# jkk-research/urban_road_filter

Hardware: NVIDIA H100
Metric: scans_per_sec (higher is better)
Workload: dtype f32/f64

## Files before the change

urban_road_filter_b200/csrc/urf_api.cu:

```cuda
#include <algorithm>
#include <cmath>
#include <cstdio>
#include <cstdlib>
#include <cstring>
#include <string>
#include <vector>

#include "urf_kernels.cuh"
#include "urf_host.hpp"
#include "urf_queue_internal.hpp"

using namespace urf;

constexpr int kMaxBatch = 65535;

struct urf_ctx {
  int device = 0;
  int max_points = 0;
  int max_batch = 0;
  size_t P = 0;
  int Tmax = 0;
  cudaStream_t stream = nullptr;
  cudaStream_t s_in = nullptr, s_out = nullptr;
  static constexpr int kGroups = 16;
  cudaStream_t s_grp[kGroups] = {};
  cudaEvent_t ev_fork = nullptr, ev_join[kGroups] = {};
  cudaStream_t s_side[kGroups + 1] = {};
  cudaEvent_t ev_sfork[kGroups + 1] = {}, ev_sjoin[kGroups + 1] = {};
  int sort_ctas = 0;
  int groups = 2;
  bool use_graph = true;
  cudaGraphExec_t gexec = nullptr;
  int g_B = -1, g_S = -1, g_order = -1, g_launches = 0;
  unsigned long long g_version = 0, version = 1;
  std::vector<cudaEvent_t> ev_in, ev_comp;
  cudaEvent_t ev0 = nullptr, ev1 = nullptr;
  DevBuffers buf{};
  struct HostSlot {
    float4* in = nullptr;
    unsigned char* rawb = nullptr;
    size_t rawb_bytes = 0;
    int* n = nullptr;
    int* label = nullptr;
    signed char* label8 = nullptr;
    int* order = nullptr;
    int* ring = nullptr;
    ScanOut* out = nullptr;
    int* h_n = nullptr;
    ScanOut* h_out = nullptr;
    cudaEvent_t ev0 = nullptr, ev1 = nullptr;
    cudaEvent_t ev_done = nullptr;
    int batch = 0, S = 0, launches = 0;
    urf_result* outs = nullptr;
    urf_clouds* clouds = nullptr;
  };
  HostSlot hs[2];
  int hs_head = 0, hs_count = 0;
  float4* pack = nullptr;
  int* packcnt = nullptr;
  int* packtot = nullptr;
  int tie_order = URF_TIES_INPUT_ORDER;
  int* h_packtot = nullptr;
  urf_params params{};
  DevParams dp{};
  static constexpr int kNRing = 8;
  int* h_nring = nullptr;
  cudaEvent_t ev_nring[kNRing] = {};
  int nring_pos = 0;
  int last_B = 0, last_S = 0;
  int launches = 0;
  float last_ms = 0.f;
  bool timing_valid = false, timing_host = false;
  std::string err;
  std::vector<void*> allocs;
  bool profile = false;
  int kslots = 1, kslot = 0;
  std::vector<cudaEvent_t> kev;
  std::vector<const char*> knames;
  std::vector<int> kcounts;
  int kcount = 0;
};

namespace {

int cuda_rc(urf_ctx* ctx, cudaError_t e, const char* call) {
  if (e == cudaSuccess) return URF_OK;
  ctx->err = std::string(call) + ": " + cudaGetErrorString(e);
  return e == cudaErrorMemoryAllocation ? URF_ERR_NOMEM : URF_ERR_CUDA;
}

#define CK(call)                                                                                   \
  do {                                                                                             \
    const int rc_ = cuda_rc(ctx, (call), #call);                                                   \
    if (rc_ != URF_OK) return rc_;                                                                 \
  } while (0)

template <class T> int dalloc(urf_ctx* ctx, T** p, size_t count) {
  void* q = nullptr;
  CK(cudaMalloc(&q, count * sizeof(T) + 256));
  ctx->allocs.push_back(q);
  CK(cudaMemsetAsync(q, 0, count * sizeof(T) + 256, ctx->stream));
  CK(cudaStreamSynchronize(ctx->stream));
  *p = static_cast<T*>(q);
  return URF_OK;
}

__global__ void k_ring32(DevBuffers buf, int* dst, int S) {
  const int b = blockIdx.y, i = blockIdx.x * blockDim.x + threadIdx.x;
  if (i < buf.n[b]) dst[(size_t)b * S + i] = max((int)buf.ringid[(size_t)b * S + i], -1);
}

DevBuffers offset_view(const DevBuffers& a, int b0, int S, int T, int channels) {
  DevBuffers v = a;
  const size_t o = (size_t)b0 * S;
  v.in += o; v.label += o; v.order += o; v.n += b0; v.out += b0;
  if (v.epos) { v.epos += o; v.lomuto += (size_t)b0 * (kRingKeys + 1); }
  if (v.label8) v.label8 += o;
  v.alpha_v += o; v.mark += o; v.ringid += o; v.sect += o; v.bpt += o;
  v.sr += o; v.sz += o; v.sidx += o; v.ssrz += o; v.ssl += o;
  v.az += o; v.d2 += o; v.baz += o; v.roadlist += o; v.roadcnt += (size_t)b0 * ((S + 31) >> 5); v.sortbuf += 2 * o;
  v.Tf += (size_t)b0 * channels * kTStride; v.Tb += (size_t)b0 * channels * kTStride;
  v.lut += (size_t)b0 * (kElevBins + 1); v.firstidx += (size_t)b0 * (kElevBins + 1);
  v.hist += (size_t)b0 * T * channels;
  v.cmin += (size_t)b0 * channels * kDegBins; v.cmax += (size_t)b0 * channels * kDegBins;
  v.ne += (size_t)b0 * channels * (kDegBins + 1);
  v.tab += b0;
  return v;
}

constexpr int kMaxKernels = 32;
constexpr int kMarkSingleMax = 300000;
thread_local std::string g_create_err;

int launch_pipeline(urf_ctx* ctx, const DevBuffers& buf, int B, int S, bool want_order, int group, int* launched) {
  DevParams dp = ctx->dp;
  const bool ref = ctx->tie_order == URF_TIES_REFERENCE;
  dp.want_order = want_order || ref ? 1 : 0;
  cudaStream_t st = group < urf_ctx::kGroups ? ctx->s_grp[group] : ctx->stream;
  const int T = (S + kChunk - 1) / kChunk;
  if (T > ctx->Tmax) return URF_ERR_CAPACITY;
  int L = 0;
  ctx->kcount = 0;
  const dim3 gpts((S + 255) / 256, B), gchunk((T + kWarpsPerBlock - 1) / kWarpsPerBlock, B);
#define K(name, ...)                                                                         \
  do {                                                                                       \
    if (ctx->profile && ctx->kcount < kMaxKernels) {                                         \
      ctx->knames[ctx->kcount] = name;                                                       \
      CK(cudaEventRecord(ctx->kev[(size_t)ctx->kslot * (kMaxKernels + 1) + ctx->kcount], st)); \
      ctx->kcount++;                                                                         \
    }                                                                                        \
    __VA_ARGS__;                                                                             \
    L++;                                                                                     \
  } while (0)
  K("k_reset", k_reset<<<dim3(8, B), 256, 0, st>>>(buf, dp));
  K("k_points", k_points<<<gpts, 256, 0, st>>>(buf, dp, S));
  K("k_register", k_register<<<B, 256, 0, st>>>(buf, dp, S));
  K("k_assign", k_assign<<<gchunk, kWarpsPerBlock * 32, 0, st>>>(buf, dp, S, T));
  K("k_scan_offsets", k_scan_offsets<<<B, kScanOffThreads, 0, st>>>(buf, dp, S, T));
  K("k_scatter", k_scatter<<<dim3((T + kScatterWarps - 1) / kScatterWarps, B), kScatterWarps * 32, kScatterSmem, st>>>(buf, dp, S, T));
  const bool fork = dp.star && !ctx->profile;
  cudaStream_t st_ring = fork ? ctx->s_side[group] : st;
  if (fork) {
    CK(cudaEventRecord(ctx->ev_sfork[group], st));
    CK(cudaStreamWaitEvent(st_ring, ctx->ev_sfork[group], 0));
  }
  if (dp.curbPoints == 5)
    K("k_ring_detect4", k_ring_detect4<<<dim3((S + kTile4 - 1) / kTile4, B), 256, 0, st_ring>>>(buf, dp, S));
  else K("k_ring_detect", k_ring_detect<<<gpts, 256, 0, st_ring>>>(buf, dp, S));
  if (fork) CK(cudaEventRecord(ctx->ev_sjoin[group], st_ring));
  if (dp.star) {
    const int gbig = std::max(4, std::min(kSectKeys, 2048 / B));
    const dim3 gscan((kSectKeys + kScanWarps * 32 - 1) / (kScanWarps * 32), B);
    const int gsort = std::min(ctx->sort_ctas, (B * kSectKeys + kSortWarps - 1) / kSortWarps);
    K("k_star_sort", k_star_sort<<<gsort, kSortWarps * 32, kStarSortSmem, st>>>(buf, dp, S, B));
    K("k_star_sort_big", k_star_sort_big<<<dim3(gbig, B), 256, kStarCtaSmem, st>>>(buf, dp, S));
    K("k_star_scan", k_star_scan<<<gscan, kScanWarps * 32, 0, st>>>(buf, dp, S));
    if (dp.star_prefix)
      K("k_star_refine", k_star_refine<<<dim3(std::max(8, std::min(kSectKeys / 8, 8192 / B)), B), 256, kStarCtaSmem, st>>>(buf, dp, S));
  }
  if (fork) CK(cudaStreamWaitEvent(st, ctx->ev_sjoin[group], 0));
  K("k_tab1", k_tab1<<<dim3((dp.channels + 7) / 8, B), 256, 0, st>>>(buf, dp));
  K("k_reach", k_reach<<<dim3((2 * kDegBins + 7) / 8, B), 256, 0, st>>>(buf, dp));
  K("k_tab2", k_tab2<<<dim3((dp.channels + kTab2Rings - 1) / kTab2Rings, B), kTab2Rings * 64, 0, st>>>(buf, dp));
  const dim3 glabel((S + kLabelThreads * kLabelGroups - 1) / (kLabelThreads * kLabelGroups), B), gsort(dp.channels, B);
  if (ref) {
    K("k_sort_rings", k_sort_rings<true><<<gsort, kSortThreads, kRingSmemKeys * sizeof(unsigned long long), st>>>(buf, S));
    K("k_lomuto_rings", k_lomuto_rings<<<gsort, kLomutoThreads, kLomutoSmem, st>>>(buf, S));
    K("k_label", k_label<true><<<glabel, kLabelThreads, 0, st>>>(buf, dp, S));
  } else K("k_label", k_label<false><<<glabel, kLabelThreads, 0, st>>>(buf, dp, S));
  if (S > kMarkSingleMax) {
    const dim3 gm(std::max(1, std::min(64, S / 16384)), B);
    K("k_markers_grid1", k_markers_grid<1><<<gm, kMarkGridThreads, 0, st>>>(buf, S));
    K("k_markers_grid2", k_markers_grid<2><<<gm, kMarkGridThreads, 0, st>>>(buf, S));
    if (ref) K("k_verts", k_verts<true><<<B, 384, 0, st>>>(buf, S));
    else K("k_verts", k_verts<false><<<B, 384, 0, st>>>(buf, S));
  } else if (ref) K("k_markers1", k_markers1<true><<<dim3(1, B), kMark1Threads, 0, st>>>(buf, S));
  else K("k_markers1", k_markers1<false><<<dim3(1, B), kMark1Threads, 0, st>>>(buf, S));
  if (want_order && !ref) K("k_sort_rings", k_sort_rings<false><<<gsort, kSortThreads, kRingSmemKeys * sizeof(unsigned long long), st>>>(buf, S));
#undef K
  if (ctx->profile) {
    CK(cudaEventRecord(ctx->kev[(size_t)ctx->kslot * (kMaxKernels + 1) + kMaxKernels], st));
    ctx->kcounts[ctx->kslot] = ctx->kcount;
    ctx->kslot = (ctx->kslot + 1) % ctx->kslots;
  }
  CK(cudaGetLastError());
  *launched = L;
  return URF_OK;
}

int update_graph(urf_ctx* ctx, int B, int S, bool want_order) {
  if (ctx->gexec && ctx->g_B == B && ctx->g_S == S && ctx->g_order == (int)want_order && ctx->g_version == ctx->version) return URF_OK;
  if (ctx->gexec) { cudaGraphExecDestroy(ctx->gexec); ctx->gexec = nullptr; }
  cudaGraph_t graph = nullptr;
  CK(cudaStreamBeginCapture(ctx->stream, cudaStreamCaptureModeThreadLocal));
  int L = 0;
  const int rc = launch_pipeline(ctx, ctx->buf, B, S, want_order, urf_ctx::kGroups, &L);
  const cudaError_t e = cudaStreamEndCapture(ctx->stream, &graph);
  if (rc != URF_OK || e != cudaSuccess || !graph) { if (graph) cudaGraphDestroy(graph); ctx->err = "graph capture failed"; return rc != URF_OK ? rc : URF_ERR_CUDA; }
  const cudaError_t ei = cudaGraphInstantiate(&ctx->gexec, graph, 0);
  cudaGraphDestroy(graph);
  if (ei != cudaSuccess) { ctx->gexec = nullptr; ctx->err = cudaGetErrorString(ei); return URF_ERR_CUDA; }
  ctx->g_B = B; ctx->g_S = S; ctx->g_order = (int)want_order; ctx->g_version = ctx->version; ctx->g_launches = L;
  return URF_OK;
}

void fill_result(const ScanOut& o, urf_result* r, bool with_ring_start) {
  r->n_in = o.n_in; r->n_roi = o.n_roi;
  r->flags = o.flags & F_PUBLIC_MASK; r->reserved = 0;
  if (o.n_roi < 30) {
    r->status = URF_TOO_FEW_POINTS;
    r->n_rings = 0; r->n_order = 0; r->n_road = 0; r->n_curb = 0; r->n_vert = 0;
    if (with_ring_start && r->ring_start) for (int k = 0; k <= URF_MAX_CHANNELS; k++) r->ring_start[k] = 0;
    return;
  }
  r->status = URF_OK;
  r->n_rings = o.n_rings; r->n_order = o.n_order; r->n_road = o.n_road; r->n_curb = o.n_curb; r->n_vert = o.n_vert;
  std::memcpy(r->vert, o.vert, sizeof(float) * 4 * (size_t)o.n_vert);
  if (with_ring_start && r->ring_start) std::memcpy(r->ring_start, o.ring_start, sizeof(int) * (URF_MAX_CHANNELS + 1));
}

}

extern "C" {

int urf_version(void) { return URF_VERSION; }

const char* urf_strerror(int code) {
  switch (code) {
    case URF_OK: return "ok";
    case URF_TOO_FEW_POINTS: return "fewer than 30 points in the ROI: nothing published";
    case URF_ERR_INVALID: return "invalid argument";
    case URF_ERR_NO_DEVICE: return "no CUDA device (this library has no CPU fallback)";
    case URF_ERR_CUDA: return "CUDA error";
    case URF_ERR_NOMEM: return "out of device or pinned memory";
    case URF_ERR_CAPACITY: return "scan or batch larger than the context was created for";
    case URF_ERR_TIMEOUT: return "timed out";
    case URF_ERR_CLOSED: return "queue closed";
    default: return "unknown error";
  }
}

const char* urf_last_cuda_error(const urf_ctx* ctx) {
  if (ctx) return ctx->err.c_str();
  return g_create_err.empty() ? "null context" : g_create_err.c_str();
}

void urf_default_params(urf_params* p) {
  if (!p) return;
  std::memset(p, 0, sizeof(*p));
  std::snprintf(p->fixed_frame, sizeof(p->fixed_frame), "left_os1/os1_lidar");
  std::snprintf(p->topic_name, sizeof(p->topic_name), "/left_os1/os1_cloud_node/points");
  p->x_zero_method = 1; p->z_zero_method = 1; p->star_shaped_method = 1; p->blind_spots = 1; p->xDirection = 0;
  p->interval = 0.18; p->curb_height = 0.05; p->curb_points = 5; p->beamZone = 30;
  p->min_x = 0; p->max_x = 30; p->min_y = -10; p->max_y = 10; p->min_z = -3; p->max_z = -1;
  p->cylinder_deg_x = 150; p->cylinder_deg_z = 140; p->curb_slope_deg = 50;
  p->kdev_param = 1.225; p->kdist_param = 2; p->starbeam_filter = 0; p->dmin_param = 10;
  p->simple_poly_allow = 1; p->poly_s_param = 0.7; p->poly_z_manual = -1.5; p->poly_z_avg_allow = 1;
  p->channels = 64;
}

int urf_create(urf_ctx** out, int device, int max_points, int max_batch) {
  if (!out || max_points < 1 || max_batch < 1 || max_points > (1 << 24)) return URF_ERR_INVALID;
  if ((long long)(max_points + kChunk) * max_batch >= (1ll << 31)) return URF_ERR_CAPACITY;
  if (max_batch > kMaxBatch) return URF_ERR_CAPACITY;
  *out = nullptr;
  int ndev = 0;
  if (cudaGetDeviceCount(&ndev) != cudaSuccess || ndev <= 0 || device < 0 || device >= ndev) return URF_ERR_NO_DEVICE;
  urf_ctx* ctx = new urf_ctx();
  auto fail = [&](int rc) { g_create_err = ctx->err.empty() ? std::string(urf_strerror(rc)) : ctx->err; urf_destroy(ctx); return rc; };
  ctx->device = device;
  if (cudaSetDevice(device) != cudaSuccess) return fail(URF_ERR_NO_DEVICE);
  ctx->max_points = ((max_points + kChunk - 1) / kChunk) * kChunk;
  ctx->max_batch = max_batch;
  ctx->P = (size_t)ctx->max_points * max_batch;
  ctx->Tmax = ctx->max_points / kChunk;
  int rc;
#define TRY(x) do { rc = (x); if (rc != URF_OK) return fail(rc); } while (0)
#define CKF(call) do { cudaError_t e_ = (call); if (e_ != cudaSuccess) { ctx->err = cudaGetErrorString(e_); return fail(URF_ERR_CUDA); } } while (0)
  CKF(cudaStreamCreateWithFlags(&ctx->stream, cudaStreamNonBlocking));
  CKF(cudaStreamCreateWithFlags(&ctx->s_in, cudaStreamNonBlocking));
  CKF(cudaStreamCreateWithFlags(&ctx->s_out, cudaStreamNonBlocking));
  for (int g = 0; g < urf_ctx::kGroups; g++) {
    CKF(cudaStreamCreateWithFlags(&ctx->s_grp[g], cudaStreamNonBlocking));
    CKF(cudaEventCreateWithFlags(&ctx->ev_join[g], cudaEventDisableTiming));
  }
  CKF(cudaEventCreateWithFlags(&ctx->ev_fork, cudaEventDisableTiming));
  for (int g = 0; g <= urf_ctx::kGroups; g++) {
    CKF(cudaStreamCreateWithFlags(&ctx->s_side[g], cudaStreamNonBlocking));
    CKF(cudaEventCreateWithFlags(&ctx->ev_sfork[g], cudaEventDisableTiming));
    CKF(cudaEventCreateWithFlags(&ctx->ev_sjoin[g], cudaEventDisableTiming));
  }
  CKF(cudaEventCreate(&ctx->ev0));
  CKF(cudaEventCreate(&ctx->ev1));
  const size_t P = ctx->P;
  DevBuffers& b = ctx->buf;
  urf_ctx::HostSlot& h0 = ctx->hs[0];
  TRY(dalloc(ctx, &h0.in, P));
  h0.rawb_bytes = (size_t)ctx->max_points * URF_MAX_POINT_STEP;
  TRY(dalloc(ctx, &h0.rawb, h0.rawb_bytes));
  TRY(dalloc(ctx, &b.alpha_v, P));
  TRY(dalloc(ctx, &b.mark, P));
  TRY(dalloc(ctx, &b.ringid, P));
  TRY(dalloc(ctx, &b.sect, P));
  TRY(dalloc(ctx, &h0.label, P));
  TRY(dalloc(ctx, &b.bpt, P));
  TRY(dalloc(ctx, &b.sr, P));
  TRY(dalloc(ctx, &b.sz, P));
  TRY(dalloc(ctx, &b.sidx, P));
  TRY(dalloc(ctx, &b.ssrz, P));
  TRY(dalloc(ctx, &b.ssl, P));
  TRY(dalloc(ctx, &b.az, P));
  TRY(dalloc(ctx, &b.d2, P));
  TRY(dalloc(ctx, &b.baz, P));
  TRY(dalloc(ctx, &b.roadlist, P));
  TRY(dalloc(ctx, &b.roadcnt, P / 32 + (size_t)max_batch + 1));
  TRY(dalloc(ctx, &b.Tf, (size_t)max_batch * kTStride * URF_MAX_CHANNELS));
  TRY(dalloc(ctx, &b.Tb, (size_t)max_batch * kTStride * URF_MAX_CHANNELS));
  TRY(dalloc(ctx, &b.lut, (size_t)max_batch * (kElevBins + 1)));
  TRY(dalloc(ctx, &b.order, P));
  TRY(dalloc(ctx, &b.sortbuf, 2 * P));
  TRY(dalloc(ctx, &b.hist, (size_t)max_batch * ctx->Tmax * kRingKeys));
  TRY(dalloc(ctx, &b.firstidx, (size_t)max_batch * (kElevBins + 1)));
  TRY(dalloc(ctx, &b.cmin, (size_t)max_batch * URF_MAX_CHANNELS * kDegBins));
  TRY(dalloc(ctx, &b.cmax, (size_t)max_batch * URF_MAX_CHANNELS * kDegBins));
  TRY(dalloc(ctx, &b.ne, (size_t)max_batch * URF_MAX_CHANNELS * (kDegBins + 1)));
  TRY(dalloc(ctx, &b.newY, (size_t)ctx->max_points));
  TRY(dalloc(ctx, &b.n, (size_t)max_batch));
  TRY(dalloc(ctx, &b.out, (size_t)max_batch));
  TRY(dalloc(ctx, &b.tab, (size_t)max_batch));
  b.in = h0.in;
  b.label = h0.label;
  h0.n = b.n; h0.order = b.order; h0.out = b.out;
  h0.ring = reinterpret_cast<int*>(b.sortbuf);
  CKF(cudaMallocHost((void**)&h0.h_n, sizeof(int) * max_batch));
  CKF(cudaMallocHost((void**)&ctx->h_nring, sizeof(int) * max_batch * urf_ctx::kNRing));
  for (int r = 0; r < urf_ctx::kNRing; r++) CKF(cudaEventCreateWithFlags(&ctx->ev_nring[r], cudaEventDisableTiming));
  CKF(cudaMallocHost((void**)&h0.h_out, sizeof(ScanOut) * max_batch));
  CKF(cudaEventCreate(&h0.ev0));
  CKF(cudaEventCreate(&h0.ev1));
  CKF(cudaEventCreateWithFlags(&h0.ev_done, cudaEventDisableTiming));
  {
    std::vector<float> ny;
    host_newY(ny, ctx->max_points);
    CKF(cudaMemcpy(b.newY, ny.data(), sizeof(float) * ny.size(), cudaMemcpyHostToDevice));
    float bd[kSectKeys], bo[kSectKeys], Kfi;
    unsigned char byx[kSectKeys];
    host_beam_init(bd, bo, byx, &Kfi);
    CKF(cudaMemcpyToSymbol(c_beam_d, bd, sizeof(bd)));
    CKF(cudaMemcpyToSymbol(c_beam_o, bo, sizeof(bo)));
    CKF(cudaMemcpyToSymbol(c_beam_yx, byx, sizeof(byx)));
    ctx->dp.Kfi = Kfi;
  }
  CKF(cudaFuncSetAttribute(k_star_sort, cudaFuncAttributeMaxDynamicSharedMemorySize, (int)kStarSortSmem));
  {
    int sms = 0, per_sm = 0;
    CKF(cudaDeviceGetAttribute(&sms, cudaDevAttrMultiProcessorCount, ctx->device));
    CKF(cudaOccupancyMaxActiveBlocksPerMultiprocessor(&per_sm, k_star_sort, kSortWarps * 32, kStarSortSmem));
    ctx->sort_ctas = std::max(1, sms * per_sm);
  }
  CKF(cudaFuncSetAttribute(k_star_sort_big, cudaFuncAttributeMaxDynamicSharedMemorySize, (int)kStarCtaSmem));
  CKF(cudaFuncSetAttribute(k_star_refine, cudaFuncAttributeMaxDynamicSharedMemorySize, (int)kStarCtaSmem));
  CKF(cudaFuncSetAttribute(k_scatter, cudaFuncAttributeMaxDynamicSharedMemorySize, (int)kScatterSmem));
  CKF(cudaFuncSetAttribute(k_scatter, cudaFuncAttributePreferredSharedMemoryCarveout, (int)cudaSharedmemCarveoutMaxShared));
  CKF(cudaFuncSetAttribute(k_sort_rings<false>, cudaFuncAttributeMaxDynamicSharedMemorySize, (int)(kRingSmemKeys * sizeof(unsigned long long))));
  CKF(cudaFuncSetAttribute(k_sort_rings<true>, cudaFuncAttributeMaxDynamicSharedMemorySize, (int)(kRingSmemKeys * sizeof(unsigned long long))));
  CKF(cudaFuncSetAttribute(k_lomuto_rings, cudaFuncAttributeMaxDynamicSharedMemorySize, (int)kLomutoSmem));
  urf_default_params(&ctx->params);
  const char* fe = std::getenv("URF_FORCE_EXACT_REGISTRATION");
  narrow_params(&ctx->params, &ctx->dp, ctx->dp.Kfi, fe && fe[0] == '1', 0);
  ctx->dp.star_prefix = 1;
  ctx->dp.star_pivot = 17;
#undef TRY
#undef CKF
  *out = ctx;
  return URF_OK;
}

void urf_destroy(urf_ctx* ctx) {
  if (!ctx) return;
  cudaSetDevice(ctx->device);
  for (cudaStream_t s : {ctx->s_in, ctx->stream, ctx->s_out}) if (s) cudaStreamSynchronize(s);
  for (void* p : ctx->allocs) cudaFree(p);
  if (ctx->h_nring) cudaFreeHost(ctx->h_nring);
  for (cudaEvent_t e : ctx->ev_nring) if (e) cudaEventDestroy(e);
  for (urf_ctx::HostSlot& h : ctx->hs) {
    if (h.h_n) cudaFreeHost(h.h_n);
    if (h.h_out) cudaFreeHost(h.h_out);
    for (cudaEvent_t e : {h.ev0, h.ev1, h.ev_done}) if (e) cudaEventDestroy(e);
  }
  if (ctx->h_packtot) cudaFreeHost(ctx->h_packtot);
  if (ctx->gexec) cudaGraphExecDestroy(ctx->gexec);
  for (cudaEvent_t e : ctx->kev) cudaEventDestroy(e);
  for (cudaEvent_t e : ctx->ev_in) cudaEventDestroy(e);
  for (cudaEvent_t e : ctx->ev_comp) cudaEventDestroy(e);
  for (int g = 0; g < urf_ctx::kGroups; g++) { if (ctx->s_grp[g]) cudaStreamDestroy(ctx->s_grp[g]); if (ctx->ev_join[g]) cudaEventDestroy(ctx->ev_join[g]); }
  if (ctx->ev_fork) cudaEventDestroy(ctx->ev_fork);
  for (int g = 0; g <= urf_ctx::kGroups; g++) {
    if (ctx->s_side[g]) cudaStreamDestroy(ctx->s_side[g]);
    if (ctx->ev_sfork[g]) cudaEventDestroy(ctx->ev_sfork[g]);
    if (ctx->ev_sjoin[g]) cudaEventDestroy(ctx->ev_sjoin[g]);
  }
  if (ctx->s_in) cudaStreamDestroy(ctx->s_in);
  if (ctx->s_out) cudaStreamDestroy(ctx->s_out);
  if (ctx->ev0) cudaEventDestroy(ctx->ev0);
  if (ctx->ev1) cudaEventDestroy(ctx->ev1);
  if (ctx->stream) cudaStreamDestroy(ctx->stream);
  delete ctx;
}

void* urf_pinned_alloc(size_t bytes) {
  void* p = nullptr;
  if (cudaHostAlloc(&p, bytes ? bytes : 1, cudaHostAllocPortable) != cudaSuccess) { cudaGetLastError(); return nullptr; }
  return p;
}
void urf_pinned_free(void* p) { if (p) cudaFreeHost(p); }

int urf_set_params(urf_ctx* ctx, const urf_params* p) {
  if (!ctx || !p || ctx->hs_count) return URF_ERR_INVALID;
  int rc = validate_params(p);
  if (rc != URF_OK) return rc;
  ctx->params = *p;
  narrow_params(p, &ctx->dp, ctx->dp.Kfi, ctx->dp.force_exact, 0);
  ctx->version++;
  return URF_OK;
}

int urf_get_params(const urf_ctx* ctx, urf_params* p) {
  if (!ctx || !p) return URF_ERR_INVALID;
  *p = ctx->params;
  return URF_OK;
}

int urf_set_option(urf_ctx* ctx, int option, int value) {
  if (!ctx || ctx->hs_count) return URF_ERR_INVALID;
  CK(cudaSetDevice(ctx->device));
  ctx->version++;
  if (option == 0) { ctx->dp.force_exact = value != 0; ctx->version++; return URF_OK; }
  if (option == 4) { ctx->dp.star_prefix = value != 0; ctx->version++; return URF_OK; }
  if (option == 3) { ctx->use_graph = value != 0; return URF_OK; }
  if (option == 2) { ctx->groups = value < 1 ? 1 : (value > urf_ctx::kGroups ? urf_ctx::kGroups : value); return URF_OK; }
  if ((option >= 5 && option <= 9) || option == 11 || option == 12) return URF_OK;
  if (option == 10) { ctx->dp.star_pivot = value < 3 ? 3 : (value > 28 ? 28 : value); return URF_OK; }
  if (option == 1) {
    CK(cudaStreamSynchronize(ctx->stream));
    if (ctx->gexec) { cudaGraphExecDestroy(ctx->gexec); ctx->gexec = nullptr; ctx->g_B = -1; }
    for (cudaEvent_t e : ctx->kev) cudaEventDestroy(e);
    ctx->kev.clear();
    ctx->profile = value > 0;
    ctx->kslots = value > 0 ? value : 1;
    ctx->kslot = 0;
    if (ctx->profile) {
      ctx->kev.assign((size_t)ctx->kslots * (kMaxKernels + 1), nullptr);
      for (cudaEvent_t& e : ctx->kev) {
        const cudaError_t ce = cudaEventCreate(&e);
        if (ce != cudaSuccess) {
          for (cudaEvent_t f : ctx->kev) if (f) cudaEventDestroy(f);
          ctx->kev.clear(); ctx->profile = false; ctx->kslots = 1;
          ctx->err = std::string("cudaEventCreate: ") + cudaGetErrorString(ce);
          return URF_ERR_CUDA;
        }
      }
      ctx->knames.assign(kMaxKernels, "");
      ctx->kcounts.assign(ctx->kslots, 0);
    }
    return URF_OK;
  }
  return URF_ERR_INVALID;
}

int urf_set_tie_order(urf_ctx* ctx, int mode) {
  if (!ctx || ctx->hs_count || (mode != URF_TIES_INPUT_ORDER && mode != URF_TIES_REFERENCE)) return URF_ERR_INVALID;
  CK(cudaSetDevice(ctx->device));
  if (mode == URF_TIES_REFERENCE && !ctx->buf.lomuto) {
    int* epos = nullptr;
    int* lomuto = nullptr;
    int rc = dalloc(ctx, &epos, ctx->P);
    if (rc == URF_OK) rc = dalloc(ctx, &lomuto, (size_t)ctx->max_batch * (kRingKeys + 1));
    if (rc != URF_OK) return rc;
    ctx->buf.epos = epos;
    ctx->buf.lomuto = lomuto;
  }
  ctx->tie_order = mode;
  ctx->version++;
  return URF_OK;
}

int urf_get_tie_order(const urf_ctx* ctx, int* mode) {
  if (!ctx || !mode) return URF_ERR_INVALID;
  *mode = ctx->tie_order;
  return URF_OK;
}

int urf_mq_set_tie_order(urf_mq* mq, int mode) {
  if (!mq || (mode != URF_TIES_INPUT_ORDER && mode != URF_TIES_REFERENCE)) return URF_ERR_INVALID;
  return urf_internal::mq_apply_idle(mq, [](urf_ctx* c, const void* m) { return urf_set_tie_order(c, *static_cast<const int*>(m)); }, &mode);
}

void* urf_stream(urf_ctx* ctx) { return ctx ? (void*)ctx->stream : nullptr; }

float urf_last_device_ms(const urf_ctx* c) {
  urf_ctx* ctx = const_cast<urf_ctx*>(c);
  if (!ctx || !ctx->timing_valid) return -1.f;
  if (ctx->timing_host) return ctx->last_ms;
  float ms = -1.f;
  if (cudaEventSynchronize(ctx->ev1) != cudaSuccess) return -1.f;
  if (cudaEventElapsedTime(&ms, ctx->ev0, ctx->ev1) != cudaSuccess) return -1.f;
  return ms;
}

int urf_last_launch_count(const urf_ctx* ctx) { return ctx ? ctx->launches : 0; }

// ... 206 lines not shown
int finish_batch(urf_ctx* ctx) {
  if (!ctx || ctx->hs_count == 0) return URF_ERR_INVALID;
  urf_ctx::HostSlot& h = ctx->hs[ctx->hs_head];
  ctx->hs_count--;
  ctx->hs_head = ctx->hs_count ? 1 - ctx->hs_head : 0;
  CK(cudaSetDevice(ctx->device));
  CK(cudaEventSynchronize(h.ev_done));
  cudaStream_t st = ctx->stream;
  urf_clouds* clouds = h.clouds;
  if (clouds) {
    const int* t = ctx->h_packtot;
    const float4 *d_rc = ctx->pack, *d_roi = ctx->pack + 2 * (size_t)ctx->max_points, *d_prob = ctx->pack + 4 * (size_t)ctx->max_points;
    clouds->n_road = t[0]; clouds->n_curb = t[1]; clouds->n_roi = t[2]; clouds->n_road_probably = t[3];
    const size_t rec = sizeof(urf_point_xyzi);
    if (clouds->road && t[0] > 0) CK(cudaMemcpyAsync(clouds->road, d_rc, rec * t[0], cudaMemcpyDeviceToHost, st));
    if (clouds->curb && t[1] > 0) CK(cudaMemcpyAsync(clouds->curb, d_rc + 2 * (size_t)t[0], rec * t[1], cudaMemcpyDeviceToHost, st));
    if (clouds->roi && t[2] > 0) CK(cudaMemcpyAsync(clouds->roi, d_roi, rec * t[2], cudaMemcpyDeviceToHost, st));
    if (clouds->road_probably && t[3] > 0) CK(cudaMemcpyAsync(clouds->road_probably, d_prob, rec * t[3], cudaMemcpyDeviceToHost, st));
    CK(cudaStreamSynchronize(st));
  }
  float ms = -1.f;
  if (cudaEventElapsedTime(&ms, h.ev0, h.ev1) != cudaSuccess) ms = -1.f;
  ctx->last_ms = ms;
  ctx->launches = h.launches;
  ctx->timing_valid = true;
  ctx->timing_host = true;
  ctx->last_B = h.batch; ctx->last_S = h.S;
  urf_result* outs = h.outs;
  for (int b = 0; b < h.batch; b++) {
    fill_result(h.h_out[b], &outs[b], true);
    if (outs[b].status == URF_TOO_FEW_POINTS && outs[b].ring) for (int i = 0; i < h.h_n[b]; i++) outs[b].ring[i] = -1;
  }
  return URF_OK;
}

int alloc_second_slot(urf_ctx* ctx) {
  urf_ctx::HostSlot& h = ctx->hs[1];
  if (h.ev_done) return URF_OK;
  CK(cudaSetDevice(ctx->device));
  const size_t P = ctx->P;
  urf_ctx::HostSlot t;
  int* ring0 = nullptr;
  int rc = dalloc(ctx, &t.in, P);
  if (rc == URF_OK) rc = dalloc(ctx, &t.label, P);
  if (rc == URF_OK) rc = dalloc(ctx, &t.order, P);
  if (rc == URF_OK) rc = dalloc(ctx, &t.ring, P);
  if (rc == URF_OK) rc = dalloc(ctx, &ring0, P);
  if (rc == URF_OK) rc = dalloc(ctx, &t.n, (size_t)ctx->max_batch);
  if (rc == URF_OK) rc = dalloc(ctx, &t.out, (size_t)ctx->max_batch);
  if (rc != URF_OK) return rc;
  if (!h.h_n) rc = cuda_rc(ctx, cudaMallocHost((void**)&h.h_n, sizeof(int) * ctx->max_batch), "cudaMallocHost");
  if (rc == URF_OK && !h.h_out) rc = cuda_rc(ctx, cudaMallocHost((void**)&h.h_out, sizeof(ScanOut) * ctx->max_batch), "cudaMallocHost");
  if (rc == URF_OK && !h.ev0) rc = cuda_rc(ctx, cudaEventCreate(&h.ev0), "cudaEventCreate");
  if (rc == URF_OK && !h.ev1) rc = cuda_rc(ctx, cudaEventCreate(&h.ev1), "cudaEventCreate");
  if (rc != URF_OK) return rc;
  h.in = t.in; h.label = t.label; h.order = t.order; h.ring = t.ring; h.n = t.n; h.out = t.out;
  ctx->hs[0].ring = ring0;
  return cuda_rc(ctx, cudaEventCreateWithFlags(&h.ev_done, cudaEventDisableTiming), "cudaEventCreate");
}

int process_batch_impl(urf_ctx* ctx, const void* const* data, const int* n, int batch, int step, int ox, int oy, int oz, int oi,
                       urf_result* outs, int8_t* const* label8, urf_clouds* clouds) {
  if (ctx && ctx->hs_count) return URF_ERR_INVALID;
  const int rc = enqueue_batch(ctx, data, n, batch, step, ox, oy, oz, oi, outs, label8, clouds);
  return rc != URF_OK ? rc : finish_batch(ctx);
}

int enqueue_async(urf_ctx* ctx, const void* const* data, const int* n, int batch, int step, int ox, int oy, int oz, int oi,
                  urf_result* outs, int8_t* const* label8) {
  if (!ctx) return URF_ERR_INVALID;
  const int rc = alloc_second_slot(ctx);
  return rc != URF_OK ? rc : enqueue_batch(ctx, data, n, batch, step, ox, oy, oz, oi, outs, label8, nullptr);
}
}

int urf_enqueue_batch(urf_ctx* ctx, const float* const* xyzi, const int* n, int batch, urf_result* outs, int8_t* const* label8) {
  return enqueue_async(ctx, reinterpret_cast<const void* const*>(xyzi), n, batch, 0, 0, 0, 0, -1, outs, label8);
}

int urf_enqueue_cloud2_batch(urf_ctx* ctx, const void* const* data, const int* n_points, int batch, int point_step, int off_x, int off_y,
                             int off_z, int off_intensity, urf_result* outs, int8_t* const* label8) {
  if (point_step == 0) return URF_ERR_INVALID;
  return enqueue_async(ctx, data, n_points, batch, point_step, off_x, off_y, off_z, off_intensity, outs, label8);
}

int urf_finish_batch(urf_ctx* ctx) { return finish_batch(ctx); }

int urf_process_batch(urf_ctx* ctx, const float* const* xyzi, const int* n, int batch, urf_result* outs) {
  return process_batch_impl(ctx, reinterpret_cast<const void* const*>(xyzi), n, batch, 0, 0, 0, 0, -1, outs, nullptr, nullptr);
}

int urf_process_batch_xyz(urf_ctx* ctx, const float* const* xyz, const int* n, int batch, urf_result* outs, int8_t* const* label8) {
  return process_batch_impl(ctx, reinterpret_cast<const void* const*>(xyz), n, batch, 12, 0, 4, 8, -1, outs, label8, nullptr);
}

int urf_process_cloud2_batch(urf_ctx* ctx, const void* const* data, const int* n_points, int batch, int point_step, int off_x, int off_y,
                             int off_z, int off_intensity, urf_result* outs, int8_t* const* label8) {
  if (point_step == 0) return URF_ERR_INVALID;
  return process_batch_impl(ctx, data, n_points, batch, point_step, off_x, off_y, off_z, off_intensity, outs, label8, nullptr);
}

int urf_process_cloud2(urf_ctx* ctx, const void* data, int n, int point_step, int off_x, int off_y, int off_z, urf_result* out) {
  if (point_step == 0) return URF_ERR_INVALID;
  return process_batch_impl(ctx, &data, &n, 1, point_step, off_x, off_y, off_z, -1, out, nullptr, nullptr);
}

int urf_process_cloud2_packed(urf_ctx* ctx, const void* data, int n, int point_step, int off_x, int off_y, int off_z,
                              int off_intensity, urf_result* out, urf_clouds* clouds) {
  if (!clouds || point_step == 0) return URF_ERR_INVALID;
  return process_batch_impl(ctx, &data, &n, 1, point_step, off_x, off_y, off_z, off_intensity, out, nullptr, clouds);
}

int urf_process(urf_ctx* ctx, const float* xyzi, int n, urf_result* out) {
  const float* ptrs[1] = {xyzi};
  return urf_process_batch(ctx, ptrs, &n, 1, out);
}

int urf_test_math(int device, int which, const float* a, const float* b, float* out, int n) {
  if (cudaSetDevice(device) != cudaSuccess) return URF_ERR_NO_DEVICE;
  float *da = nullptr, *db = nullptr, *dout = nullptr;
  if (cudaMalloc(&da, sizeof(float) * n) != cudaSuccess || cudaMalloc(&db, sizeof(float) * n) != cudaSuccess ||
      cudaMalloc(&dout, sizeof(float) * n) != cudaSuccess)
    return URF_ERR_NOMEM;
  cudaMemcpy(da, a, sizeof(float) * n, cudaMemcpyHostToDevice);
  cudaMemcpy(db, b ? b : a, sizeof(float) * n, cudaMemcpyHostToDevice);
  k_test_math<<<(n + 255) / 256, 256>>>(da, db, dout, n, which);
  cudaError_t e = cudaMemcpy(out, dout, sizeof(float) * n, cudaMemcpyDeviceToHost);
  cudaFree(da); cudaFree(db); cudaFree(dout);
  return e == cudaSuccess ? URF_OK : URF_ERR_CUDA;
}

int urf_debug_fetch(urf_ctx* ctx, int b, int what, void* dst, size_t bytes) {
  if (!ctx || !dst || b < 0 || b >= ctx->last_B) return URF_ERR_INVALID;
  CK(cudaSetDevice(ctx->device));
  CK(cudaStreamSynchronize(ctx->stream));
  const size_t off = (size_t)b * ctx->last_S;
  const void* src = nullptr;
  switch (what) {
    case 0: src = ctx->buf.alpha_v + off; break;
    case 1: src = ctx->buf.mark + off; break;
    case 2: src = ctx->buf.ringid + off; break;
    case 3: src = ctx->buf.sect + off; break;
    case 4: src = ctx->buf.az + off; break;
    case 5: src = ctx->buf.d2 + off; break;
    case 8: src = ctx->buf.tab + b; if (bytes > sizeof(ScanTab)) bytes = sizeof(ScanTab); break;
    case 9: src = &ctx->buf.tab[b].nbig; if (bytes > 2 * sizeof(int)) bytes = 2 * sizeof(int); break;
    case 10: src = &ctx->buf.tab[b].nrefine; if (bytes > sizeof(int)) bytes = sizeof(int); break;
    case 11: case 12: {
      const size_t ch = (size_t)ctx->dp.channels;
      src = (what == 11 ? ctx->buf.Tf : ctx->buf.Tb) + (size_t)b * ch * kTStride;
      if (bytes > sizeof(float) * ch * kDegBins) bytes = sizeof(float) * ch * kDegBins;
      break;
    }
    default: return URF_ERR_INVALID;
  }
  CK(cudaMemcpy(dst, src, bytes, cudaMemcpyDeviceToHost));
  return URF_OK;
}

size_t urf_debug_sizeof_tab(void) { return sizeof(ScanTab); }

}
```

urban_road_filter_b200/csrc/urf_kernels.cuh:

```cuda
#pragma once
#include <type_traits>

#include "urf_device.cuh"
#include "urf_logic.cuh"
#include "urf_lomuto.cuh"
#include "urf_stdsort.cuh"

namespace urf {

__constant__ float c_beam_d[kSectKeys];
__constant__ float c_beam_o[kSectKeys];
__constant__ unsigned char c_beam_yx[kSectKeys];

__device__ __forceinline__ int lane_id() { return threadIdx.x & 31; }
__device__ __forceinline__ unsigned scan_base(int b, int S) { return (unsigned)b * (unsigned)S; }

struct CtaGroup {
  static __device__ __forceinline__ unsigned rank() { return threadIdx.x; }
  static __device__ __forceinline__ unsigned size() { return blockDim.x; }
  static __device__ __forceinline__ void sync() { __syncthreads(); }
  static __device__ __forceinline__ bool any(bool p) { return __syncthreads_or(p); }
};
struct WarpGroup {
  static __device__ __forceinline__ int rank() { return lane_id(); }
  static __device__ __forceinline__ int size() { return 32; }
  static __device__ __forceinline__ void sync() { __syncwarp(); }
  static __device__ __forceinline__ bool any(bool p) { return __any_sync(0xffffffffu, p); }
};

template <class G, class T>
__device__ void group_bitonic(T* a, int npad) {
  for (int k = 2; k <= npad; k <<= 1) {
    for (int j = k >> 1; j > 0; j >>= 1) {
      for (int t = G::rank(); t < (npad >> 1); t += G::size()) {
        int i = 2 * t - (t & (j - 1));
        int l = i + j;
        bool up = (i & k) == 0;
        T x = a[i], y = a[l];
        if ((x > y) == up) { a[i] = y; a[l] = x; }
      }
      G::sync();
    }
  }
}

__device__ __forceinline__ int next_pow2(int n) { int p = 1; while (p < n) p <<= 1; return p; }

__device__ __forceinline__ void curb_hit(const DevBuffers& buf, const DevParams& prm, int b, unsigned gb, int idx, int k) {
  buf.mark[gb + (unsigned)idx] = 2;
  if (k < 0) k = buf.ringid[gb + (unsigned)idx];
  if (k < 0) return;
  const float a = buf.az[gb + (unsigned)idx];
  if (a >= 0.0f) {
    const unsigned o = ((unsigned)b * (unsigned)prm.channels + (unsigned)k) * kDegBins + (unsigned)deg_bin(a);
    atomicMin(&buf.cmin[o], fbits(a));
    atomicMax(&buf.cmax[o], fbits(a));
  }
}
__device__ __forceinline__ int ring_of_position(const int* __restrict__ ring_start, int p) {
  int lo = 0, hi = kRingKeys;
  while (lo < hi) { const int mid = (lo + hi) >> 1; if (ring_start[mid] <= p) lo = mid + 1; else hi = mid; }
  return lo - 1;
}

__global__ void k_reset(DevBuffers buf, DevParams prm) {
  const int b = blockIdx.y;
  const int tid = blockIdx.x * blockDim.x + threadIdx.x;
  const int nth = gridDim.x * blockDim.x;
  ScanOut& o = buf.out[b];
  ScanTab& t = buf.tab[b];
  if (tid == 0) {
    o.n_in = buf.n[b]; o.n_roi = 0; o.n_rings = 0; o.n_order = 0; o.n_road = 0; o.n_curb = 0; o.n_vert = 0; o.flags = 0;
  }
  for (int i = tid; i <= kRingKeys; i += nth) o.ring_start[i] = 0;
  for (int i = tid; i < kRingKeys; i += nth) { t.maxs[i] = 0ull; t.maxdist[i] = 0u; t.angle[i] = 0.f; t.regidx[i] = 0x7fffffff; t.regorder[i] = 0x7fffffff; }
  for (int i = tid; i < kDegBins; i += nth) { t.cutbest[i] = ~0ull; t.dmax[i] = 0u; t.best[i] = ~0ull; }
  for (int i = tid; i < kSectKeys; i += nth) t.sect_cnt[i] = 0;
  if (tid == 0) { t.nbig = 0; t.nslow = 0; t.nrefine = 0; }
  if (tid == 0 && buf.lomuto) buf.lomuto[(size_t)b * (kRingKeys + 1)] = 0;
  unsigned* fi = buf.firstidx + (size_t)b * (kElevBins + 1);
  for (int i = tid; i <= kElevBins; i += nth) fi[i] = 0xffffffffu;
  const size_t nb = (size_t)prm.channels * kDegBins;
  unsigned* cmin = buf.cmin + (size_t)b * nb;
  unsigned* cmax = buf.cmax + (size_t)b * nb;
  for (size_t i = tid; i < nb; i += nth) { cmin[i] = 0x7f800000u; cmax[i] = 0u; }
}

__global__ void __launch_bounds__(256) k_points(DevBuffers buf, DevParams prm, int S) {
  const int b = blockIdx.y;
  const int n = buf.n[b];
  const int i = blockIdx.x * blockDim.x + threadIdx.x;
  int keep = 0, sec = -1;
  if (i < n) {
    const unsigned g = scan_base(b, S) + (unsigned)i;
    const float4 p = __ldg(&buf.in[g]);
    keep = roi_keep(prm, p.x, p.y, p.z);
    float a = -1.0f;
    if (keep) {
      float d, az;
      point_angles(p.x, p.y, p.z, &a, &d, &az);
      unsigned* fi = buf.firstidx + (size_t)b * (kElevBins + 1) + elev_bin(a);
      if (*fi > (unsigned)i) atomicMin(fi, (unsigned)i);
      if (a == 0.0f) atomicOr(&buf.out[b].flags, F_ZERO_ALPHA);
      if (az != az) atomicOr(&buf.out[b].flags, F_NAN_AZIMUTH);
      if (prm.star) sec = star_sector(prm, p.x, p.y, c_beam_d, c_beam_o, c_beam_yx);
      buf.az[g] = az;
      buf.d2[g] = d;
    }
    buf.alpha_v[g] = a;
    buf.mark[g] = 0;
    buf.sect[g] = (short)sec;
  }
  const unsigned bal = __ballot_sync(0xffffffffu, keep);
  if (lane_id() == 0 && bal) atomicAdd(&buf.out[b].n_roi, __popc(bal));
  const unsigned peers = __match_any_sync(0xffffffffu, sec);
  if (sec >= 0 && lane_id() == __ffs(peers) - 1) atomicAdd(&buf.tab[b].sect_cnt[sec], __popc(peers));
}

__device__ void register_exact_cta(const float* __restrict__ alpha, int n, float interval, int channels, float* s_vis,
                                   float* s_reg, int* s_idx, int* s_red, int* out_m) {
  __shared__ int s_min;
  int m = 0, vis = 0, i_last = -1;
  bool frozen = false;
  while (m < channels) {
    int local = 0x7fffffff;
    for (int i = i_last + 1 + threadIdx.x; i < n; i += blockDim.x) {
      const float a = alpha[i];
      if (a < 0.0f) continue;
      bool cov = false;
      for (int t = 0; t < vis; t++) {
        if (fabsf(__fsub_rn(s_vis[t], a)) <= interval) { cov = true; break; }
      }
      if (!cov) { local = i; break; }
    }
    for (int o = 16; o > 0; o >>= 1) local = min(local, __shfl_xor_sync(0xffffffffu, local, o));
    if (lane_id() == 0) s_red[threadIdx.x >> 5] = local;
    __syncthreads();
    if (threadIdx.x == 0) {
      int v = 0x7fffffff;
      for (int w = 0; w < (int)(blockDim.x >> 5); w++) v = min(v, s_red[w]);
      s_min = v;
    }
    __syncthreads();
    const int istar = s_min;
    __syncthreads();
    if (istar == 0x7fffffff) break;
    const float a = alpha[istar];
    if (threadIdx.x == 0) { s_reg[m] = a; s_idx[m] = istar; if (!frozen && a != 0.0f) s_vis[vis] = a; }
    if (!frozen) { if (a == 0.0f) frozen = true; else vis++; }
    m++;
    i_last = istar;
    __syncthreads();
  }
  *out_m = m;
}

__device__ void publish_rings_cta(ScanTab& tab, ScanOut& out, unsigned short* lut, float interval, const float* s_reg,
                                  const int* s_idx, int m, unsigned long long* s_keys, float* s_sorted) {
  for (int t = threadIdx.x; t < kRingKeys; t += blockDim.x)
    s_keys[t] = t < m ? (((unsigned long long)fbits(s_reg[t]) << 32) | (unsigned)s_idx[t]) : ~0ull;
  __syncthreads();
  group_bitonic<CtaGroup>(s_keys, kRingKeys);
  for (int t = threadIdx.x; t < kRingKeys; t += blockDim.x) {
    if (t < m) {
      const float a = bitsf((unsigned)(s_keys[t] >> 32));
      s_sorted[t] = a;
      tab.angle[t] = a;
      tab.regidx[t] = (int)(unsigned)s_keys[t];
      tab.regorder[t] = s_idx[t];
    } else { s_sorted[t] = 0.f; tab.angle[t] = 0.f; tab.regidx[t] = 0x7fffffff; tab.regorder[t] = 0x7fffffff; }
  }
  if (threadIdx.x == 0) out.n_rings = m;
  __syncthreads();
  for (int e = threadIdx.x; e <= kElevBins; e += blockDim.x) lut[e] = (unsigned short)ring_lut_entry(s_sorted, m, interval, e);
}

__global__ void __launch_bounds__(256) k_register(DevBuffers buf, DevParams prm, int S) {
  const int b = blockIdx.x;
  const int n = buf.n[b];
  ScanOut& out = buf.out[b];
  ScanTab& tab = buf.tab[b];
  const float* alpha = buf.alpha_v + (size_t)b * S;
  __shared__ unsigned s_cand[kMaxCand];
  __shared__ float s_calpha[kMaxCand];
  __shared__ float s_vis[kRingKeys];
  __shared__ float s_reg[kRingKeys];
  __shared__ float s_sorted[kRingKeys];
  __shared__ int s_idx[kRingKeys];
  __shared__ unsigned long long s_keys[kRingKeys];
  __shared__ int s_red[8];
  __shared__ int s_cnt, s_m;
  if (out.n_roi < 30) {
    if (threadIdx.x == 0) out.n_rings = 0;
    return;
  }
  bool exact = prm.force_exact || (out.flags & F_ZERO_ALPHA);
  if (!exact) {
    if (threadIdx.x == 0) s_cnt = 0;
    __syncthreads();
    const unsigned* fi = buf.firstidx + (size_t)b * (kElevBins + 1);
    for (int t = threadIdx.x; t <= kElevBins; t += blockDim.x) {
      const unsigned v = fi[t];
      if (v != 0xffffffffu) { int s = atomicAdd(&s_cnt, 1); if (s < kMaxCand) s_cand[s] = v; }
    }
    __syncthreads();
    const int cnt = s_cnt;
    if (cnt > kMaxCand) exact = true;
    else {
      const int npad = next_pow2(cnt < 2 ? 2 : cnt);
      for (int t = cnt + threadIdx.x; t < npad; t += blockDim.x) s_cand[t] = 0xffffffffu;
      __syncthreads();
      group_bitonic<CtaGroup>(s_cand, npad);
      for (int t = threadIdx.x; t < cnt; t += blockDim.x) s_calpha[t] = alpha[s_cand[t]];
      __syncthreads();
      if (threadIdx.x < 32) {
        int m = 0;
        for (int c = 0; c < cnt && m < prm.channels; c++) {
          const float a = s_calpha[c];
          bool cov = false;
          for (int t = lane_id(); t < m; t += 32)
            if (fabsf(__fsub_rn(s_reg[t], a)) <= prm.interval) cov = true;
          cov = __any_sync(0xffffffffu, cov);
          if (!cov) {
            if (lane_id() == 0) { s_reg[m] = a; s_idx[m] = (int)s_cand[c]; }
            m++;
            __syncwarp();
          }
        }
        if (lane_id() == 0) s_m = m;
      }
      __syncthreads();
    }
  }
  if (exact) {
    int m;
    register_exact_cta(alpha, n, prm.interval, prm.channels, s_vis, s_reg, s_idx, s_red, &m);
    if (threadIdx.x == 0) { s_m = m; atomicOr(&out.flags, F_EXACT_REG); }
    __syncthreads();
  }
  publish_rings_cta(tab, out, buf.lut + (size_t)b * (kElevBins + 1), prm.interval, s_reg, s_idx, s_m, s_keys, s_sorted);
}

__device__ __forceinline__ bool assign_chunk(const DevBuffers& buf, const DevParams& prm, int b, int S, int T, int chunk, int n, bool live,
                                             bool verify, const float* s_angle, const int* s_regidx, const int* regorder, int R,
                                             const unsigned short* __restrict__ lut, unsigned* cnt, int lane) {
  bool violation = false;
  constexpr int H = 8;
  static_assert((kChunk / 32) % H == 0, "chunk iterations come in groups of H");
#pragma unroll 1
  for (int h0 = 0; h0 < kChunk / 32; h0 += H) {
    float av[H];
    unsigned short start[H];
#pragma unroll
    for (int u = 0; u < H; u++) {
      const int i = chunk * kChunk + (h0 + u) * 32 + lane;
      av[u] = i < n ? buf.alpha_v[scan_base(b, S) + (unsigned)i] : -1.0f;
    }
#pragma unroll
    for (int u = 0; u < H; u++) start[u] = (live && av[u] >= 0.0f) ? lut[elev_bin(av[u])] : (unsigned short)0;
#pragma unroll
    for (int u = 0; u < H; u++) {
      const int i = chunk * kChunk + (h0 + u) * 32 + lane;
      int ring = -1;
      if (i < n) {
        const float a = av[u];
        const bool kept = live && a >= 0.0f;
        if (kept) {
          int lo;
          ring = assign_ring_from(s_angle, R, a, prm.interval, start[u], &lo);
// ... 1667 lines not shown
```

Measured before the change: 81980.

## Make k_points persistent with shared-memory privatized atomics and prefetch

k_points now launches an occupancy-sized grid in which each block walks a contiguous range of tiles, two points per thread, with register double-buffered prefetch of the next tile's input. The firstidx min, per-sector counts and ROI count are accumulated in shared memory and flushed to global with one atomic per bin per block. The aim is to cut global atomic contention and launch/tail overhead. In exchange each block pays per-block init and flush of the shared bins, and a small debug readback case for firstidx is added.

```diff
diff --git a/urban_road_filter_b200/csrc/urf_api.cu b/urban_road_filter_b200/csrc/urf_api.cu
--- a/urban_road_filter_b200/csrc/urf_api.cu
+++ b/urban_road_filter_b200/csrc/urf_api.cu
@@ -28,6 +28,7 @@
   cudaStream_t s_side[kGroups + 1] = {};
   cudaEvent_t ev_sfork[kGroups + 1] = {}, ev_sjoin[kGroups + 1] = {};
   int sort_ctas = 0;
+  int pts_ctas = 0;
   int groups = 2;
   bool use_graph = true;
   cudaGraphExec_t gexec = nullptr;
@@ -153,7 +154,8 @@
     L++;                                                                                     \
   } while (0)
   K("k_reset", k_reset<<<dim3(8, B), 256, 0, st>>>(buf, dp));
-  K("k_points", k_points<<<gpts, 256, 0, st>>>(buf, dp, S));
+  const int gp = std::max(1, std::min(ctx->pts_ctas / B, (S + kPtsTile - 1) / kPtsTile));
+  K("k_points", k_points<<<dim3(gp, B), kPtsThreads, 0, st>>>(buf, dp, S));
   K("k_register", k_register<<<B, 256, 0, st>>>(buf, dp, S));
   K("k_assign", k_assign<<<gchunk, kWarpsPerBlock * 32, 0, st>>>(buf, dp, S, T));
   K("k_scan_offsets", k_scan_offsets<<<B, kScanOffThreads, 0, st>>>(buf, dp, S, T));
@@ -377,6 +379,8 @@
     CKF(cudaDeviceGetAttribute(&sms, cudaDevAttrMultiProcessorCount, ctx->device));
     CKF(cudaOccupancyMaxActiveBlocksPerMultiprocessor(&per_sm, k_star_sort, kSortWarps * 32, kStarSortSmem));
     ctx->sort_ctas = std::max(1, sms * per_sm);
+    CKF(cudaOccupancyMaxActiveBlocksPerMultiprocessor(&per_sm, k_points, kPtsThreads, 0));
+    ctx->pts_ctas = std::max(1, sms * per_sm);
   }
   CKF(cudaFuncSetAttribute(k_star_sort_big, cudaFuncAttributeMaxDynamicSharedMemorySize, (int)kStarCtaSmem));
   CKF(cudaFuncSetAttribute(k_star_refine, cudaFuncAttributeMaxDynamicSharedMemorySize, (int)kStarCtaSmem));
@@ -889,6 +893,10 @@
       if (bytes > sizeof(float) * ch * kDegBins) bytes = sizeof(float) * ch * kDegBins;
       break;
     }
+    case 13:
+      src = ctx->buf.firstidx + (size_t)b * (kElevBins + 1);
+      if (bytes > sizeof(unsigned) * (kElevBins + 1)) bytes = sizeof(unsigned) * (kElevBins + 1);
+      break;
     default: return URF_ERR_INVALID;
   }
   CK(cudaMemcpy(dst, src, bytes, cudaMemcpyDeviceToHost));
diff --git a/urban_road_filter_b200/csrc/urf_kernels.cuh b/urban_road_filter_b200/csrc/urf_kernels.cuh
--- a/urban_road_filter_b200/csrc/urf_kernels.cuh
+++ b/urban_road_filter_b200/csrc/urf_kernels.cuh
@@ -86,35 +86,81 @@
   for (size_t i = tid; i < nb; i += nth) { cmin[i] = 0x7f800000u; cmax[i] = 0u; }
 }
 
-__global__ void __launch_bounds__(256) k_points(DevBuffers buf, DevParams prm, int S) {
+constexpr int kPtsThreads = 256;
+constexpr int kPtsPerThread = 2;
+constexpr int kPtsTile = kPtsThreads * kPtsPerThread;
+__global__ void __launch_bounds__(kPtsThreads) k_points(DevBuffers buf, DevParams prm, int S) {
+  __shared__ unsigned s_first[kElevBins + 1];
+  __shared__ int s_scnt[kSectKeys];
+  __shared__ int s_roi;
   const int b = blockIdx.y;
   const int n = buf.n[b];
-  const int i = blockIdx.x * blockDim.x + threadIdx.x;
-  int keep = 0, sec = -1;
-  if (i < n) {
-    const unsigned g = scan_base(b, S) + (unsigned)i;
-    const float4 p = __ldg(&buf.in[g]);
-    keep = roi_keep(prm, p.x, p.y, p.z);
-    float a = -1.0f;
-    if (keep) {
-      float d, az;
-      point_angles(p.x, p.y, p.z, &a, &d, &az);
-      unsigned* fi = buf.firstidx + (size_t)b * (kElevBins + 1) + elev_bin(a);
-      if (*fi > (unsigned)i) atomicMin(fi, (unsigned)i);
-      if (a == 0.0f) atomicOr(&buf.out[b].flags, F_ZERO_ALPHA);
-      if (az != az) atomicOr(&buf.out[b].flags, F_NAN_AZIMUTH);
-      if (prm.star) sec = star_sector(prm, p.x, p.y, c_beam_d, c_beam_o, c_beam_yx);
-      buf.az[g] = az;
-      buf.d2[g] = d;
-    }
-    buf.alpha_v[g] = a;
-    buf.mark[g] = 0;
-    buf.sect[g] = (short)sec;
-  }
-  const unsigned bal = __ballot_sync(0xffffffffu, keep);
-  if (lane_id() == 0 && bal) atomicAdd(&buf.out[b].n_roi, __popc(bal));
-  const unsigned peers = __match_any_sync(0xffffffffu, sec);
-  if (sec >= 0 && lane_id() == __ffs(peers) - 1) atomicAdd(&buf.tab[b].sect_cnt[sec], __popc(peers));
+  const int tiles = (n + kPtsTile - 1) / kPtsTile;
+  const int per = (tiles + gridDim.x - 1) / gridDim.x;
+  const int t0 = blockIdx.x * per, t1 = min(tiles, t0 + per);
+  if (t0 >= t1) return;
+  for (int e = threadIdx.x; e <= kElevBins; e += kPtsThreads) s_first[e] = 0xffffffffu;
+  for (int s = threadIdx.x; s < kSectKeys; s += kPtsThreads) s_scnt[s] = 0;
+  if (threadIdx.x == 0) s_roi = 0;
+  const unsigned gb = scan_base(b, S);
+  float4 cur[kPtsPerThread], nxt[kPtsPerThread];
+#pragma unroll
+  for (int j = 0; j < kPtsPerThread; ++j) {
+    const int i = t0 * kPtsTile + j * kPtsThreads + (int)threadIdx.x;
+    if (i < n) cur[j] = __ldg(&buf.in[gb + (unsigned)i]);
+  }
+  __syncthreads();
+  int roi = 0;
+  for (int t = t0; t < t1; ++t) {
+    if (t + 1 < t1) {
+#pragma unroll
+      for (int j = 0; j < kPtsPerThread; ++j) {
+        const int i = (t + 1) * kPtsTile + j * kPtsThreads + (int)threadIdx.x;
+        if (i < n) nxt[j] = __ldg(&buf.in[gb + (unsigned)i]);
+      }
+    }
+#pragma unroll
+    for (int j = 0; j < kPtsPerThread; ++j) {
+      const int i = t * kPtsTile + j * kPtsThreads + (int)threadIdx.x;
+      int sec = -1;
+      if (i < n) {
+        const unsigned g = gb + (unsigned)i;
+        const float4 p = cur[j];
+        const int keep = roi_keep(prm, p.x, p.y, p.z);
+        float a = -1.0f;
+        if (keep) {
+          float d, az;
+          point_angles(p.x, p.y, p.z, &a, &d, &az);
+          unsigned* fi = s_first + elev_bin(a);
+          if (*fi > (unsigned)i) atomicMin(fi, (unsigned)i);
+          if (a == 0.0f) atomicOr(&buf.out[b].flags, F_ZERO_ALPHA);
+          if (az != az) atomicOr(&buf.out[b].flags, F_NAN_AZIMUTH);
+          if (prm.star) sec = star_sector(prm, p.x, p.y, c_beam_d, c_beam_o, c_beam_yx);
+          buf.az[g] = az;
+          buf.d2[g] = d;
+          roi++;
+        }
+        buf.alpha_v[g] = a;
+        buf.mark[g] = 0;
+        buf.sect[g] = (short)sec;
+      }
+      const unsigned peers = __match_any_sync(0xffffffffu, sec);
+      if (sec >= 0 && lane_id() == __ffs(peers) - 1) atomicAdd(&s_scnt[sec], __popc(peers));
+    }
+#pragma unroll
+    for (int j = 0; j < kPtsPerThread; ++j) cur[j] = nxt[j];
+  }
+  roi = __reduce_add_sync(0xffffffffu, roi);
+  if (lane_id() == 0 && roi) atomicAdd(&s_roi, roi);
+  __syncthreads();
+  unsigned* fi = buf.firstidx + (size_t)b * (kElevBins + 1);
+  for (int e = threadIdx.x; e <= kElevBins; e += kPtsThreads) {
+    const unsigned v = s_first[e];
+    if (v != 0xffffffffu) atomicMin(&fi[e], v);
+  }
+  for (int s = threadIdx.x; s < kSectKeys; s += kPtsThreads)
+    if (s_scnt[s]) atomicAdd(&buf.tab[b].sect_cnt[s], s_scnt[s]);
+  if (threadIdx.x == 0 && s_roi) atomicAdd(&buf.out[b].n_roi, s_roi);
 }
 
 __device__ void register_exact_cta(const float* __restrict__ alpha, int n, float interval, int channels, float* s_vis,
```

Measured after the change: 88500, median of 6. 8.0% higher.
